# parthjaggi/flow

Measured on AMD Instinct MI355X. Metric: env-steps/sec, higher is better.
Workload: dtype mixed

## Files before the change

flow_amd/csrc/flowsim.hip:

```cpp
#include "flowsim_sim.h"

namespace fsim {

int validate(const fs_config* c) {
  if (!c) return fail(FS_ERR_INVALID, "fs_create: cfg is NULL");
  if (c->struct_size != sizeof(fs_config))
    return fail(FS_ERR_INVALID, "fs_create: struct_size mismatch (header/library out of sync)");
  if (c->abi_version != FS_ABI_VERSION) return fail(FS_ERR_INVALID, "fs_create: abi_version mismatch");
  if (c->precision != FS_F32 && c->precision != FS_F64 && c->precision != FS_MIXED && c->precision != FS_F16S)
    return fail(FS_ERR_INVALID, "fs_create: bad precision");
  if (c->precision == FS_F16S && (c->network != FS_NET_MERGE || c->num_vehicles > 64))
    return fail(FS_ERR_UNSUPPORTED, "fs_create: FS_F16S (half state, float32 integrator) is built for FS_NET_MERGE "
                                    "(k_steps_open, <= 64 vehicle slots)");
  if (c->precision == FS_MIXED && (c->network == FS_NET_MERGE || c->network == FS_NET_BOTTLENECK)) {
  } else if (c->precision == FS_MIXED) {
    const bool fig8 = c->network == FS_NET_FIGURE_EIGHT;
    const char* why = nullptr;
    if ((c->network != FS_NET_RING && !fig8) || c->num_lanes > 1) why = "network (single-lane ring or figure eight)";
    else if (c->env != FS_ENV_ACCEL && c->env != FS_ENV_WAVE_ATTENUATION_PO) why = "env (AccelEnv or WaveAttenuationPOEnv)";
    else if (c->evaluate) why = "evaluate";
    else if (c->sims_per_step != 1) why = "sims_per_step (1)";
    else if (c->integrator != FS_EULER) why = "integrator (Euler)";
    else if (c->junction_mode && !fig8) why = "junction_mode";
    else if (c->track_aux && !fig8) why = "track_aux (the scalar Env's previous-speed / acceleration fields: VecFlowEnv(track_aux=False))";
// ... 334 lines not shown
  return FS_OK;
}

int fs_use_own_stream(fs_handle h) {
  if (!h) return fail(FS_ERR_INVALID, "fs_use_own_stream: NULL handle");
  SimBase* s = S(h);
  DeviceGuard guard(s->cfg.device);
  HIP_TRY(hipStreamSynchronize(s->stream));
  s->stream = s->own_stream;
  return FS_OK;
}

int fs_sync(fs_handle h) {
  if (!h) return fail(FS_ERR_INVALID, "fs_sync: NULL handle");
  DeviceGuard guard(S(h)->cfg.device);
  HIP_TRY(hipStreamSynchronize(S(h)->stream));
  return S(h)->check_qflag();
}

int fs_reset_dev(fs_handle h, const uint8_t* mask_dev, float* obs_dev) {
  if (!h) return fail(FS_ERR_INVALID, "fs_reset_dev: NULL handle");
  SimBase* s = S(h);
  DeviceGuard guard(s->cfg.device);
  int rc = s->launch_reset(mask_dev);
  if (rc) return rc;
  float* obs = obs_dev ? obs_dev : s->d_obs;
  if (s->cfg.network == FS_NET_MERGE || s->cfg.network == FS_NET_BOTTLENECK) {
    s->after_reset = 1;
    rc = s->launch_steps(0, mask_dev, nullptr, 0, obs, s->d_rew, s->d_done, 0);
    s->after_reset = 0;
    if (rc) return rc;
    if (s->cfg.warmup_steps > 0)
      return s->launch_steps(s->cfg.warmup_steps, mask_dev, nullptr, 0, obs, s->d_rew, s->d_done, 0);
    return FS_OK;
  }
  if (s->cfg.warmup_steps > 0)
    return s->launch_steps(s->cfg.warmup_steps, mask_dev, nullptr, 0, obs, s->d_rew, s->d_done, 0);
  return s->launch_steps(0, mask_dev, nullptr, 0, obs, s->d_rew, s->d_done, 0);
}

int fs_reset(fs_handle h, const uint8_t* mask, float* obs_out) {
  if (!h) return fail(FS_ERR_INVALID, "fs_reset: NULL handle");
  SimBase* s = S(h);
  DeviceGuard guard(s->cfg.device);
  const size_t R = size_t(s->cfg.num_replicas);
  const uint8_t* dmask = nullptr;
  if (mask) {
    HIP_TRY(hipMemcpyAsync(s->d_mask, mask, R, hipMemcpyHostToDevice, s->stream));
    dmask = s->d_mask;
// ... 118 lines not shown
```

flow_amd/csrc/flowsim_kernels.h:

```cpp
#pragma once
#include <hip/hip_runtime.h>
#include <stdint.h>

#include "flowsim.h"

namespace fs {

enum : int {
  FLAG_NEED_FOLLOWER = 1,
  FLAG_NEED_MEAN = 2,
  FLAG_HAS_NOISE = 4,
  FLAG_HAS_LAC = 8,
  FLAG_NEED_SUMO = 16,
  FLAG_HAS_FAILSAFE = 32,
  FLAG_ALL_IDM = 64,
  FLAG_IDM_SET = 128,
  FLAG_NO_FLOW_CTRL = 256,
  FLAG_DELTA4 = 512,
};

template <typename T>
struct DevView {
  T* pos;
  T* vel;
// ... 1675 lines not shown
  }

  if (num_steps == 0) {
    write_obs();
    return;
  }

  if (valid && live_replica) {
    s.pos[idx] = x;
    s.vel[idx] = v;
    s.lane[idx] = ln;
    s.last_lc[idx] = last_lc;
    if (sorted) s.sort_key[idx] = xs;
    if (flags & FLAG_HAS_LAC) s.ctrl_state[idx] = cst;
    if (s.track_aux) { s.prev_vel[idx] = prev_v; s.accel[idx] = last_acc; }
    if (ii == 0) {
      s.time[rr] = tcount;
      if (flags & FLAG_HAS_NOISE) s.noise_ctr[rr] = nctr;
    }
  }
}

template <typename T>
__global__ void k_reset(DevView<T> s, const uint8_t* __restrict__ mask) {
  const size_t n = size_t(s.R) * s.N;
  for (size_t e = size_t(blockIdx.x) * blockDim.x + threadIdx.x; e < n; e += size_t(gridDim.x) * blockDim.x) {
    const int r = int(e / s.N);
    if (mask != nullptr && mask[r] == 0) continue;
    s.pos[e] = s.init_pos[e];
    s.vel[e] = s.init_vel[e];
    s.prev_vel[e] = s.init_vel[e];
    s.accel[e] = T(0);
    s.ctrl_state[e] = T(0);
    if (e % s.N == 0 && s.init_ring_len != nullptr) const_cast<T*>(s.ring_len)[r] = s.init_ring_len[r];
    if (s.sort_vehicles) {
      T xa = s.init_pos[e];
      if (s.nseg > 0) {
        bool internal;
        segment_lookup_args(s, s.init_pos[e], internal, xa);
      }
      s.sort_key[e] = xa;
    }
    if (s.num_lanes > 1 || s.env == FS_ENV_LANE_CHANGE_ACCEL || s.env == FS_ENV_LANE_CHANGE_ACCEL_PO) {
      s.lane[e] = s.init_lane[e];
      s.last_lc[e] = -(1 << 30);
    }
    if (s.n_pis > 0 && s.pis_index[e % s.N] >= 0) s.pis_n[size_t(r) * s.n_pis + s.pis_index[e % s.N]] = 0;
    if (e % s.N == 0) s.time[r] = 0;
  }
}

}
```

flow_amd/csrc/flowsim_pair.h:

```cpp
#pragma once
#include "flowsim_kernels.h"

namespace fs {

typedef float f2 __attribute__((ext_vector_type(2)));
typedef unsigned u2v __attribute__((__vector_size__(8)));

enum : int { DPP_ROW_NEWBCAST0 = 0x150, DPP_ROW_NEWBCAST8 = 0x158 };

__device__ __forceinline__ f2 fma2(f2 a, f2 b, f2 c) { return __builtin_elementwise_fma(a, b, c); }
__device__ __forceinline__ f2 splat(float a) { return f2{a, a}; }

__device__ __forceinline__ f2 pk_mul(f2 a, f2 b) { return a * b; }
__device__ __forceinline__ f2 pk_add(f2 a, f2 b) { return a + b; }
__device__ __forceinline__ f2 pk_sub(f2 a, f2 b) { return a - b; }
__device__ __forceinline__ f2 pk_fma(f2 a, f2 b, f2 c) { return fma2(a, b, c); }
__device__ __forceinline__ f2 pk_fnma(f2 a, f2 b, f2 c) { return fma2(-a, b, c); }
__device__ __forceinline__ float nonneg_else(float x, float y) {
  const unsigned a = __builtin_bit_cast(unsigned, x), b = __builtin_bit_cast(unsigned, y);
  return __builtin_bit_cast(float, min(a, b));
}

template <int ROW>
__device__ __forceinline__ float next_a(float v, bool last, int lane) {
// ... 142 lines not shown
      "v_pk_fma_f32 v[124:125], v[112:113], %[vmask], %[tvm]\n"
      "v_pk_mul_f32 v[124:125], v[124:125], v[124:125]\n"
      "v_add_f32_e32 %[sq], v124, v125\n"
      "v_cvt_f64_f32_e32 v[130:131], v112\n"
      "v_cvt_f64_f32_e32 v[132:133], v113\n"
      "v_mul_f64 v[134:135], v[130:131], %[rcms]\n"
      "v_mul_f64 v[136:137], v[132:133], %[rcms]\n"
      "v_fma_f64 v[130:131], -v[134:135], %[ms], v[130:131]\n"
      "v_fma_f64 v[132:133], -v[136:137], %[ms], v[132:133]\n"
      "v_fma_f64 v[134:135], v[130:131], %[rcms], v[134:135]\n"
      "v_fma_f64 v[136:137], v[132:133], %[rcms], v[136:137]\n"
      "v_cvt_f32_f64_e32 v128, v[134:135]\n"
      "v_cvt_f32_f64_e32 v129, v[136:137]\n"
      : "+{v[112:113]}"(V), "+{v[114:115]}"(X), "+{v[116:117]}"(H), "+{v[118:119]}"(DVL), "={v[128:129]}"(OV),
        [cb] "+v"(crash_bits), [sq] "=&v"(sq)
      : [L2] "v"(c.L2), [lenlead] "v"(c.len_lead), [gap2] "v"(c.gap2), [vmask] "v"(c.vmask), [tvm] "v"(c.tvm),
        [ms] "v"(c.ms64), [rcms] "v"(c.rc_ms64), [last] "s"(c.last_mask)
      : "v124", "v125", "v126", "v127", "v130", "v131", "v132", "v133", "v134", "v135", "v136", "v137");
}

struct MixedConsts {
  f2 p0, p1, p2, p5, rc_v0, tsab, rc_ab, one, gap2, vmask, tvm;
  float c1e3;
  double dt, ramp, L, rc_L, rc_ms, len_b, len_next, zero;
  unsigned long long last_mask;
};
__device__ __forceinline__ void mixed_step_asm_a(f2& V32, double& XA, double& XB, double& VA, double& VB, f2& H, f2& DVL,
                                                 f2& OV, const MixedConsts& c) {
  unsigned long long sa, sb;
  asm volatile(
      "v_cmp_nlt_f32_e64 %[sa], |v140|, %[c1e3]\n"
      "v_cmp_nlt_f32_e64 %[sb], |v141|, %[c1e3]\n"
      "v_pk_mul_f32 v[124:125], v[112:113], v[142:143]\n"
      "v_pk_mul_f32 v[126:127], v[124:125], %[rcab]\n"
      "v_pk_fma_f32 v[130:131], v[126:127], %[tsab], v[124:125] neg_lo:[1,0,0] neg_hi:[1,0,0]\n"
      "v_pk_fma_f32 v[126:127], v[130:131], %[rcab], v[126:127]\n"
      "v_cndmask_b32_e64 v120, %[c1e3], v140, %[sa]\n"
      "v_cndmask_b32_e64 v121, %[c1e3], v141, %[sb]\n"
      "v_pk_mul_f32 v[124:125], v[112:113], %[rcv0]\n"
      "v_rcp_f32_e32 v122, v120\n"
      "v_rcp_f32_e32 v123, v121\n"
      "v_pk_fma_f32 v[130:131], v[124:125], %[p0], v[112:113] neg_lo:[1,0,0] neg_hi:[1,0,0]\n"
      "v_pk_fma_f32 v[124:125], v[130:131], %[rcv0], v[124:125]\n"
      "v_pk_mul_f32 v[130:131], v[112:113], %[p1]\n"
      "v_pk_add_f32 v[130:131], v[130:131], v[126:127]\n"
      "v_pk_fma_f32 v[126:127], v[120:121], v[122:123], %[one] neg_lo:[1,0,0] neg_hi:[1,0,0]\n"
      "v_max_f32_e32 v130, 0, v130\n"
      "v_max_f32_e32 v131, 0, v131\n"
      "v_pk_fma_f32 v[122:123], v[126:127], v[122:123], v[122:123]\n"
      "v_pk_add_f32 v[130:131], %[p5], v[130:131]\n"
      "v_pk_mul_f32 v[124:125], v[124:125], v[124:125]\n"
// ... 3 lines not shown
      "v_pk_add_f32 v[124:125], %[one], v[124:125] neg_lo:[0,1] neg_hi:[0,1]\n"
      "v_pk_fma_f32 v[126:127], v[132:133], v[122:123], v[126:127]\n"
      "v_pk_fma_f32 v[132:133], v[120:121], v[126:127], v[130:131] neg_lo:[1,0,0] neg_hi:[1,0,0]\n"
      "v_pk_fma_f32 v[126:127], v[132:133], v[122:123], v[126:127]\n"
      "v_pk_mul_f32 v[126:127], v[126:127], v[126:127]\n"
      "v_pk_add_f32 v[124:125], v[124:125], v[126:127] neg_lo:[0,1] neg_hi:[0,1]\n"
      "v_pk_mul_f32 v[124:125], %[p2], v[124:125]\n"
      "v_cvt_f64_f32_e32 v[130:131], v124\n"
      "v_cvt_f64_f32_e32 v[132:133], v125\n"
      "v_mul_f64 v[130:131], v[130:131], %[dt]\n"
      "v_mul_f64 v[132:133], v[132:133], %[dt]\n"
      "v_add_f64 v[130:131], v[118:119], v[130:131]\n"
      "v_add_f64 v[132:133], v[138:139], v[132:133]\n"
      "v_max_f64 v[130:131], v[130:131], %[zero]\n"
      "v_max_f64 v[132:133], v[132:133], %[zero]\n"
      "v_add_f64 v[130:131], v[130:131], -v[118:119]\n"
      "v_add_f64 v[132:133], v[132:133], -v[138:139]\n"
      "v_mul_f64 v[130:131], v[130:131], %[ramp]\n"
      "v_mul_f64 v[132:133], v[132:133], %[ramp]\n"
      "v_add_f64 v[118:119], v[118:119], v[130:131]\n"
      "v_add_f64 v[138:139], v[138:139], v[132:133]\n"
      "v_mul_f64 v[130:131], v[118:119], %[dt]\n"
      "v_mul_f64 v[132:133], v[138:139], %[dt]\n"
      "v_add_f64 v[130:131], v[114:115], v[130:131]\n"
      "v_add_f64 v[132:133], v[116:117], v[132:133]\n"
      "v_add_f64 v[134:135], v[130:131], -%[L]\n"
      "v_add_f64 v[136:137], v[132:133], -%[L]\n"
      "v_cvt_f32_f64_e32 v112, v[118:119]\n"
      "v_cvt_f32_f64_e32 v113, v[138:139]\n"
      "v_cmp_gt_i32_e64 %[sa], 0, v135\n"
      "v_cmp_gt_i32_e64 %[sb], 0, v137\n"
      "v_mul_f64 v[120:121], v[118:119], %[rcms]\n"
      "v_mul_f64 v[122:123], v[138:139], %[rcms]\n"
      "v_cndmask_b32_e64 v114, v134, v130, %[sa]\n"
      "v_cndmask_b32_e64 v115, v135, v131, %[sa]\n"
      "v_cndmask_b32_e64 v116, v136, v132, %[sb]\n"
      "v_cndmask_b32_e64 v117, v137, v133, %[sb]\n"
      "v_cvt_f32_f64_e32 v128, v[120:121]\n"
      "v_cvt_f32_f64_e32 v129, v[122:123]\n"
      : "+{v[112:113]}"(V32), "+{v[114:115]}"(XA), "+{v[116:117]}"(XB), "+{v[118:119]}"(VA), "+{v[138:139]}"(VB),
        "+{v[140:141]}"(H), "+{v[142:143]}"(DVL), "={v[128:129]}"(OV), [sa] "=&s"(sa), [sb] "=&s"(sb)
      : [c1e3] "v"(c.c1e3), [rcab] "v"(c.rc_ab), [tsab] "v"(c.tsab), [rcv0] "v"(c.rc_v0), [p0] "v"(c.p0),
        [p1] "v"(c.p1), [p2] "v"(c.p2), [p5] "v"(c.p5), [one] "v"(c.one), [dt] "v"(c.dt), [ramp] "v"(c.ramp),
        [L] "v"(c.L), [rcms] "v"(c.rc_ms), [zero] "v"(c.zero)
      : "v120", "v121", "v122", "v123", "v124", "v125", "v126", "v127", "v130", "v131", "v132", "v133", "v134",
        "v135", "v136", "v137");
}
struct MixedSumoConsts { double fl0a, fl0b, adta, adtb, ddta, ddtb; };
__device__ __forceinline__ void mixed_step_asm_a_sm(f2& V32, double& XA, double& XB, double& VA, double& VB, f2& H,
                                                    f2& DVL, f2& OV, const MixedConsts& c, const SumoPair& m,
                                                    const MixedSumoConsts& d) {
  unsigned long long sa, sb;
  asm volatile(
      "v_cmp_nlt_f32_e64 %[sa], |v140|, %[c1e3]\n"
      "v_cmp_nlt_f32_e64 %[sb], |v141|, %[c1e3]\n"
      "v_pk_mul_f32 v[124:125], v[112:113], v[142:143]\n"
      "v_pk_mul_f32 v[126:127], v[124:125], %[rcab]\n"
      "v_pk_mul_f32 v[150:151], v[124:125], %[rcts]\n"
      "v_pk_fma_f32 v[130:131], v[126:127], %[tsab], v[124:125] neg_lo:[1,0,0] neg_hi:[1,0,0]\n"
      "v_pk_fma_f32 v[152:153], v[150:151], %[ts], v[124:125] neg_lo:[1,0,0] neg_hi:[1,0,0]\n"
      "v_pk_fma_f32 v[126:127], v[130:131], %[rcab], v[126:127]\n"
      "v_pk_fma_f32 v[150:151], v[152:153], %[rcts], v[150:151]\n"
      "v_cndmask_b32_e64 v120, %[c1e3], v140, %[sa]\n"
      "v_cndmask_b32_e64 v121, %[c1e3], v141, %[sb]\n"
      "v_max_f32_e32 v146, v140, %[c1e3]\n"
      "v_max_f32_e32 v147, v141, %[c1e3]\n"
      "v_pk_mul_f32 v[124:125], v[112:113], %[rcv0]\n"
      "v_rcp_f32_e32 v122, v120\n"
      "v_rcp_f32_e32 v123, v121\n"
      "v_rcp_f32_e32 v148, v146\n"
      "v_rcp_f32_e32 v149, v147\n"
      "v_pk_fma_f32 v[130:131], v[124:125], %[p0], v[112:113] neg_lo:[1,0,0] neg_hi:[1,0,0]\n"
      "v_pk_mul_f32 v[154:155], v[112:113], %[rcsm]\n"
      "v_pk_fma_f32 v[124:125], v[130:131], %[rcv0], v[124:125]\n"
// ... 49 lines not shown
      "v_add_f64 v[136:137], v[138:139], v[136:137]\n"
      "v_max_f64 v[130:131], v[130:131], %[zero]\n"
      "v_max_f64 v[132:133], v[132:133], %[zero]\n"
      "v_max_f64 v[134:135], v[134:135], %[fl0a]\n"
      "v_max_f64 v[136:137], v[136:137], %[fl0b]\n"
      "v_add_f64 v[130:131], v[130:131], -v[118:119]\n"
      "v_add_f64 v[132:133], v[132:133], -v[138:139]\n"
      "v_mul_f64 v[130:131], v[130:131], %[ramp]\n"
      "v_mul_f64 v[132:133], v[132:133], %[ramp]\n"
      "v_add_f64 v[130:131], v[118:119], v[130:131]\n"
      "v_add_f64 v[132:133], v[138:139], v[132:133]\n"
      "v_min_f64 v[130:131], v[130:131], v[134:135]\n"
      "v_min_f64 v[132:133], v[132:133], v[136:137]\n"
      "v_add_f64 v[134:135], v[118:119], %[adta]\n"
      "v_add_f64 v[136:137], v[138:139], %[adtb]\n"
      "v_min_f64 v[130:131], v[130:131], v[134:135]\n"
      "v_min_f64 v[132:133], v[132:133], v[136:137]\n"
      "v_add_f64 v[134:135], v[118:119], -%[ddta]\n"
      "v_add_f64 v[136:137], v[138:139], -%[ddtb]\n"
      "v_max_f64 v[118:119], v[130:131], v[134:135]\n"
      "v_max_f64 v[138:139], v[132:133], v[136:137]\n"
      "v_mul_f64 v[130:131], v[118:119], %[dt]\n"
      "v_mul_f64 v[132:133], v[138:139], %[dt]\n"
      "v_add_f64 v[130:131], v[114:115], v[130:131]\n"
      "v_add_f64 v[132:133], v[116:117], v[132:133]\n"
      "v_add_f64 v[134:135], v[130:131], -%[L]\n"
      "v_add_f64 v[136:137], v[132:133], -%[L]\n"
      "v_cvt_f32_f64_e32 v112, v[118:119]\n"
      "v_cvt_f32_f64_e32 v113, v[138:139]\n"
      "v_cmp_gt_i32_e64 %[sa], 0, v135\n"
      "v_cmp_gt_i32_e64 %[sb], 0, v137\n"
      "v_mul_f64 v[120:121], v[118:119], %[rcms]\n"
      "v_mul_f64 v[122:123], v[138:139], %[rcms]\n"
      "v_cndmask_b32_e64 v114, v134, v130, %[sa]\n"
      "v_cndmask_b32_e64 v115, v135, v131, %[sa]\n"
      "v_cndmask_b32_e64 v116, v136, v132, %[sb]\n"
      "v_cndmask_b32_e64 v117, v137, v133, %[sb]\n"
      "v_cvt_f32_f64_e32 v128, v[120:121]\n"
      "v_cvt_f32_f64_e32 v129, v[122:123]\n"
      : "+{v[112:113]}"(V32), "+{v[114:115]}"(XA), "+{v[116:117]}"(XB), "+{v[118:119]}"(VA), "+{v[138:139]}"(VB),
        "+{v[140:141]}"(H), "+{v[142:143]}"(DVL), "={v[128:129]}"(OV), [sa] "=&s"(sa), [sb] "=&s"(sb)
      : [c1e3] "v"(c.c1e3), [rcab] "v"(c.rc_ab), [tsab] "v"(c.tsab), [rcv0] "v"(c.rc_v0), [p0] "v"(c.p0),
        [p1] "v"(c.p1), [p2] "v"(c.p2), [p5] "v"(c.p5), [one] "v"(c.one), [dt] "v"(c.dt), [ramp] "v"(c.ramp),
        [L] "v"(c.L), [rcms] "v"(c.rc_ms), [zero] "v"(c.zero), [rcts] "v"(m.rc_ts), [ts] "v"(m.ts),
        [rcsm] "v"(m.rc_smax), [smax] "v"(m.smax), [tau] "v"(m.tau), [mgap] "v"(m.min_gap), [maxa] "v"(m.maxa),
        [fl0a] "v"(d.fl0a), [fl0b] "v"(d.fl0b), [adta] "v"(d.adta), [adtb] "v"(d.adtb), [ddta] "v"(d.ddta),
        [ddtb] "v"(d.ddtb)
      : "v120", "v121", "v122", "v123", "v124", "v125", "v126", "v127", "v130", "v131", "v132", "v133", "v134",
        "v135", "v136", "v137", "v146", "v147", "v148", "v149", "v150", "v151", "v152", "v153", "v154", "v155");
}
__device__ __forceinline__ void mixed_step_asm_b(f2& V32, double& XA, double& XB, f2& H, f2& DVL, f2& OX,
                                                 unsigned& crash_bits, float& sq, const MixedConsts& c) {
  unsigned long long sa, sb;
  asm volatile(
      "v_sub_f32_e32 v142, v112, v113\n"
      "v_subrev_f32_dpp v143, v112, v113 row_shl:1 row_mask:0xf bank_mask:0xf bound_ctrl:1\n"
      "v_subrev_f32_dpp v124, v112, v113 row_newbcast:0 row_mask:0xf bank_mask:0xf\n"
      "v_mov_b32_dpp v130, v114 row_shl:1 row_mask:0xf bank_mask:0xf bound_ctrl:1\n"
      "v_mov_b32_dpp v131, v115 row_shl:1 row_mask:0xf bank_mask:0xf bound_ctrl:1\n"
      "v_mov_b32_dpp v132, v114 row_newbcast:0 row_mask:0xf bank_mask:0xf\n"
      "v_mov_b32_dpp v133, v115 row_newbcast:0 row_mask:0xf bank_mask:0xf\n"
      "v_cndmask_b32_e64 v143, v143, v124, %[last]\n"
      "v_cndmask_b32_e64 v130, v130, v132, %[last]\n"
      "v_cndmask_b32_e64 v131, v131, v133, %[last]\n"
      "v_mul_f64 v[120:121], v[114:115], %[rcL]\n"
      "v_mul_f64 v[122:123], v[116:117], %[rcL]\n"
      "v_add_f64 v[134:135], v[116:117], -v[114:115]\n"
      "v_add_f64 v[136:137], v[130:131], -v[116:117]\n"
      "v_cvt_f32_f64_e32 v144, v[120:121]\n"
      "v_cvt_f32_f64_e32 v145, v[122:123]\n"
      "v_add_f64 v[130:131], v[134:135], %[L]\n"
      "v_add_f64 v[132:133], v[136:137], %[L]\n"
      "v_cmp_gt_i32_e64 %[sa], 0, v135\n"
      "v_cmp_gt_i32_e64 %[sb], 0, v137\n"
      "v_pk_fma_f32 v[124:125], v[112:113], %[vmask], %[tvm]\n"
      "v_pk_mul_f32 v[124:125], v[124:125], v[124:125]\n"
      "v_cndmask_b32_e64 v134, v134, v130, %[sa]\n"
      "v_cndmask_b32_e64 v135, v135, v131, %[sa]\n"
      "v_cndmask_b32_e64 v136, v136, v132, %[sb]\n"
      "v_cndmask_b32_e64 v137, v137, v133, %[sb]\n"
      "v_add_f32_e32 %[sq], v124, v125\n"
      "v_add_f64 v[134:135], v[134:135], -%[lenb]\n"
      "v_add_f64 v[136:137], v[136:137], -%[lennext]\n"
      "v_cvt_f32_f64_e32 v140, v[134:135]\n"
      "v_cvt_f32_f64_e32 v141, v[136:137]\n"
      "v_pk_add_f32 v[126:127], v[140:141], %[gap2] neg_lo:[0,1] neg_hi:[0,1]\n"
      "v_min_f32_e32 v126, v126, v127\n"
      "v_alignbit_b32 %[cb], %[cb], v126, 31\n"
      : "+{v[112:113]}"(V32), "+{v[114:115]}"(XA), "+{v[116:117]}"(XB), "+{v[140:141]}"(H), "+{v[142:143]}"(DVL),
        "={v[144:145]}"(OX), [cb] "+v"(crash_bits), [sq] "=&v"(sq), [sa] "=&s"(sa), [sb] "=&s"(sb)
      : [L] "v"(c.L), [rcL] "v"(c.rc_L), [gap2] "v"(c.gap2), [vmask] "v"(c.vmask), [tvm] "v"(c.tvm),
        [lenb] "v"(c.len_b), [lennext] "v"(c.len_next), [last] "s"(c.last_mask)
      : "v120", "v121", "v122", "v123", "v124", "v125", "v126", "v127", "v130", "v131", "v132", "v133", "v134",
        "v135", "v136", "v137");
}

template <typename T, int ROW, bool DELTA4, bool FASTDIV, bool BADCHK, bool SM = false, bool NOISE = false>
__global__ __launch_bounds__(256) void k_rollout_pair(DevView<T> s, int num_steps, float* __restrict__ obs,
                                                      float* __restrict__ rew, uint8_t* __restrict__ done) {
  constexpr bool MIXED = sizeof(T) == 8;
  static_assert(!(NOISE && MIXED), "FS_MIXED has no noise form (its C twin cannot reproduce the hardware's log / cos)");
  constexpr bool ASM = ROW == 16 && DELTA4 && FASTDIV && !BADCHK;
  constexpr int RPW = 64 / ROW;
  constexpr int PERIOD = ROW < 16 ? ROW : 16;
  const int lane = threadIdx.x & 63;
  const int wave = (blockIdx.x * blockDim.x + threadIdx.x) >> 6;
  const int row = lane / ROW;
  const int k = lane % ROW;
  const int r = wave * RPW + row;
  const int N = s.N;
  const int LP = N >> 1;
  const bool rvalid = r < s.R;
  const bool valid = rvalid && k < LP;
  const int rr = rvalid ? r : s.R - 1;
// ... 17 lines not shown
  if constexpr (NOISE) {
    if ((nctr & 3u) != 0u) {
      gauss4<float>(s.seed_lo, s.seed_hi, s.rep0 + uint32_t(rr), uint32_t(iA), nctr >> 2, gA, s.noise_exact != 0);
      gauss4<float>(s.seed_lo, s.seed_hi, s.rep0 + uint32_t(rr), uint32_t(iB), nctr >> 2, gB, s.noise_exact != 0);
      for (uint32_t q = 0; q < (nctr & 3u); ++q) {
        gA[0] = gA[1]; gA[1] = gA[2]; gA[2] = gA[3];
        gB[0] = gB[1]; gB[1] = gB[2]; gB[2] = gB[3];
      }
    }
  }

  const float dt = float(s.dt), ramp = float(s.ramp);
  const f2 two_sqrt_ab = {2.0f * tsqrt(p[2].x * p[3].x), 2.0f * tsqrt(p[2].y * p[3].y)};
  const f2 rc_v0 = {1.0f / p[0].x, 1.0f / p[0].y}, rc_ab = {1.0f / two_sqrt_ab.x, 1.0f / two_sqrt_ab.y};
  const float Lf = float(L);
  const f2 L2 = splat(Lf), rc_L2 = splat(1.0f / Lf), one = splat(1.0f), dt2 = splat(dt), ramp2 = splat(ramp);
  const f2 gap2 = splat(float(s.crash_gap)), m100 = splat(-100.0f);
  const f2 vmask = splat(valid ? 1.0f : 0.0f), tvm = splat(valid ? -float(s.target_velocity) : 0.0f);
  const double ms64 = double(s.max_speed), rc_ms64 = 1.0 / ms64;
  const double L64 = double(L), rc_L64 = 1.0 / L64, dt64 = double(s.dt), ramp64 = double(s.ramp);

  f2 x, v;
  double xdA = 0, xdB = 0, vdA = 0, vdB = 0;
  if (MIXED) {
    xdA = double(s.pos[idx]); xdB = double(s.pos[idx + 1]);
    vdA = double(s.vel[idx]); vdB = double(s.vel[idx + 1]);
    v = f2{float(vdA), float(vdB)};
    x = f2{0.0f, 0.0f};
  } else {
    x = f2{float(s.pos[idx]), float(s.pos[idx + 1])};
    v = f2{float(s.vel[idx]), float(s.vel[idx + 1])};
  }
  const f2 len_lead = {float(lenB), float(len_nextA)};

  auto headway = [&]() -> f2 {
    if (MIXED) {
      const double xn = next_a<ROW>(xdA, last, lane);
      double dA = xdB - xdA, dB = xn - xdB;
      dA = dA < 0.0 ? dA + L64 : dA;
      dB = dB < 0.0 ? dB + L64 : dB;
      return f2{float(dA - double(lenB)), float(dB - double(len_nextA))};
    } else {
      const f2 xl = {x.y, next_a<ROW>(x.x, last, lane)};
      f2 d = pk_sub(xl, x);
      const f2 dw = pk_add(d, L2);
      d.x = nonneg_else(d.x, dw.x);
      d.y = nonneg_else(d.y, dw.y);
      return pk_sub(d, len_lead);
    }
  };
  f2 h = headway();
  f2 vl = {v.y, next_a<ROW>(v.x, last, lane)};
  f2 dvl = v - vl;
  PairConsts pc;
  pc.p0 = p[0]; pc.p1 = p[1]; pc.p2 = p[2]; pc.p5 = p[5]; pc.rc_v0 = rc_v0; pc.tsab = two_sqrt_ab; pc.rc_ab = rc_ab;
  pc.one = one; pc.dt2 = dt2; pc.ramp2 = ramp2; pc.L2 = L2; pc.rc_L2 = rc_L2; pc.len_lead = len_lead;
  pc.gap2 = gap2; pc.vmask = vmask; pc.tvm = tvm; pc.c1e3 = 1e-3f; pc.ms64 = ms64; pc.rc_ms64 = rc_ms64;
  pc.last_mask = __ballot(last);
  MixedConsts mc;
  mc.p0 = p[0]; mc.p1 = p[1]; mc.p2 = p[2]; mc.p5 = p[5]; mc.rc_v0 = rc_v0; mc.tsab = two_sqrt_ab; mc.rc_ab = rc_ab;
  mc.one = one; mc.gap2 = gap2; mc.vmask = vmask; mc.tvm = tvm; mc.c1e3 = 1e-3f; mc.dt = dt64; mc.ramp = ramp64;
  mc.L = L64; mc.rc_L = rc_L64; mc.rc_ms = rc_ms64; mc.len_b = double(lenB); mc.len_next = double(len_nextA);
  mc.zero = 0.0; mc.last_mask = pc.last_mask;
  SumoPair sc{};
  double floor0A = 0, floor0B = 0, adtA = 0, adtB = 0, ddtA = 0, ddtB = 0;
  if constexpr (SM) {
    const int mA = s.speed_mode[iA], mB = s.speed_mode[iB];
    const float maA = float(s.max_accel[iA]), maB = float(s.max_accel[iB]);
    const float mdA = float(s.max_decel[iA]), mdB = float(s.max_decel[iB]);
    sc.tau = f2{float(s.sumo_tau[iA]), float(s.sumo_tau[iB])};
    sc.min_gap = f2{float(s.sumo_min_gap[iA]), float(s.sumo_min_gap[iB])};
    sc.maxa = f2{maA, maB};
    sc.smax = f2{float(s.sumo_max_speed[iA]), float(s.sumo_max_speed[iB])};
    sc.rc_smax = f2{1.0f / sc.smax.x, 1.0f / sc.smax.y};
    sc.ts = f2{2.0f * tsqrt(maA * mdA), 2.0f * tsqrt(maB * mdB)};
    sc.rc_ts = f2{1.0f / sc.ts.x, 1.0f / sc.ts.y};
    const float BIG = 3.0e38f;
    sc.floor0 = f2{(mA & 1) ? 0.0f : BIG, (mB & 1) ? 0.0f : BIG};
    sc.adt = f2{(mA & 2) ? maA * dt : BIG, (mB & 2) ? maB * dt : BIG};
    sc.ddt = f2{(mA & 4) ? mdA * dt : BIG, (mB & 4) ? mdB * dt : BIG};
    floor0A = double(sc.floor0.x); floor0B = double(sc.floor0.y);
    adtA = (mA & 2) ? double(s.max_accel[iA]) * dt64 : double(BIG);
    adtB = (mB & 2) ? double(s.max_accel[iB]) * dt64 : double(BIG);
    ddtA = (mA & 4) ? double(s.max_decel[iA]) * dt64 : double(BIG);
    ddtB = (mB & 4) ? double(s.max_decel[iB]) * dt64 : double(BIG);
  }
// ... 27 lines not shown
    if constexpr (NOISE) {
      const bool fresh = (nctr & 3u) == 0u;
      if (__ballot(fresh) != 0ull) {
        if (fresh) {
          gauss4<float>(s.seed_lo, s.seed_hi, s.rep0 + uint32_t(rr), uint32_t(iA), nctr >> 2, gA, s.noise_exact != 0);
          gauss4<float>(s.seed_lo, s.seed_hi, s.rep0 + uint32_t(rr), uint32_t(iB), nctr >> 2, gB, s.noise_exact != 0);
        }
      }
      const float tA = sigma.x * gA[0], tB = sigma.y * gB[0];
      nz.x = noisyA ? tA : -0.0f;
      nz.y = noisyB ? tB : -0.0f;
      gA[0] = gA[1]; gA[1] = gA[2]; gA[2] = gA[3];
      gB[0] = gB[1]; gB[1] = gB[2]; gB[2] = gB[3];
      nctr += 1u;
    }
    return nz;
  };

  auto one_step = [&](int slot, __amdgpu_buffer_rsrc_t rs, float& sq_out) {
    if constexpr (ASM) {
      f2 ov, ox;
      const unsigned so = unsigned(slot) * step_b32;
      if constexpr (MIXED) {
        if constexpr (SM) mixed_step_asm_a_sm(v, xdA, xdB, vdA, vdB, h, dvl, ov, mc, sc, msc);
        else mixed_step_asm_a(v, xdA, xdB, vdA, vdB, h, dvl, ov, mc);
        if (slot > 0) __builtin_amdgcn_raw_buffer_store_b128(piece, rs, off_16, so - step_b32, 0);
        mixed_step_asm_b(v, xdA, xdB, h, dvl, ox, crash_bits, sq_out, mc);
        transpose_in(ov, ox);
      } else {
#if defined(FS_DIAG_NOSTORE)
        pair_step_asm_a(v, x, h, dvl, ox, pc);
        pair_step_asm_b(v, x, h, dvl, ov, crash_bits, sq_out, pc);
        asm volatile("" :: "v"(ov), "v"(ox), "s"(so));
#elif defined(FS_DIAG_NOXPOSE)
        pair_step_asm_a(v, x, h, dvl, ox, pc);
        __builtin_amdgcn_raw_buffer_store_b64(__builtin_bit_cast(u2v, ox), rs, off_x, so, 0);
        pair_step_asm_b(v, x, h, dvl, ov, crash_bits, sq_out, pc);
        __builtin_amdgcn_raw_buffer_store_b64(__builtin_bit_cast(u2v, ov), rs, off_v, so, 0);
#else
        if constexpr (NOISE) {
          const f2 nz = noise_term();
          if constexpr (SM) pair_step_asm_a_sm_nz(v, x, h, dvl, ox, pc, sc, nz);
          else pair_step_asm_a_nz(v, x, h, dvl, ox, pc, nz);
        } else {
          if constexpr (SM) pair_step_asm_a_sm(v, x, h, dvl, ox, pc, sc);
          else pair_step_asm_a(v, x, h, dvl, ox, pc);
        }
        if (slot > 0) __builtin_amdgcn_raw_buffer_store_b128(piece, rs, off_16, so - step_b32, 0);
        pair_step_asm_b(v, x, h, dvl, ov, crash_bits, sq_out, pc);
        transpose_in(ov, ox);
// ... 149 lines not shown
```

flow_amd/csrc/flowsim_sim.h:

```cpp
#pragma once
#include <hip/hip_runtime.h>

#include <algorithm>
#include <climits>
#include <cmath>
#include <cstdio>
#include <cstdlib>
#include <cstring>
#include <map>
#include <mutex>
#include <new>
#include <string>
#include <type_traits>
#include <vector>

#include "flowsim.h"
#include "flowsim_kernels.h"
#include "flowsim_open.h"
#include "flowsim_pair.h"
#include "flowsim_fig8.h"
#include "flowsim_ringrl.h"
#include "flowsim_policy.h"
#include "flowsim_wide.h"
#include "flowsim_queue_consts.h"
// ... 68 lines not shown
  int* d_qflag = nullptr;
  bool qflag_armed = false;
  int check_qflag() {
    if (!qflag_armed || !d_qflag) return FS_OK;
    int f = 0;
    HIP_TRY(hipMemcpy(&f, d_qflag, sizeof(int), hipMemcpyDeviceToHost));
    if (f != 0)
      return fail(FS_ERR_UNSUPPORTED, "k_drop_queue: a path of the lane-drop network held more than 64 vehicles (or more than 8 "
                                      "arrived in one sub-step): the results of this handle are invalid -- create it "
                                      "with FLOWSIM_NO_QUEUE=1 (slot-order kernels)");
    qflag_armed = false;
    return FS_OK;
  }
  bool has_user_ctrl = false;
  const char* last_kernel = "";
  int launched() {
    HIP_TRY(hipGetLastError());
    return FS_OK;
  }

  virtual int launch_steps(int num_steps, const uint8_t* mask, const float* actions, size_t act_stride,
                           float* obs, float* rew, uint8_t* done, int obs_every_step) = 0;
  virtual int launch_reset(const uint8_t* mask) = 0;
  virtual int launch_policy(const fs_policy* pol, int num_steps, int reset_done, const float* obs_in, float* obs,
                            float* act, float* logp, float* rew, uint8_t* done) = 0;
  uint32_t* d_pol_ctr = nullptr;
  virtual int get_state(int field, void* dst, size_t bytes) = 0;
  virtual int set_state(int field, const void* src, size_t bytes) = 0;
  virtual int add_vehicle(int replica, int slot, int route, double x, double speed) = 0;
};

template <typename T>
struct Sim : SimBase {
  fs::DevView<T> dv{};
  fs::OpenView<T> ov{};
  fs::QueueConsts qc{};
  bool open_net = false;
  std::vector<T> h_len;
  std::vector<T> h_ring_len;

  template <typename U>
  int dev_alloc(U** out, size_t count) {
    void* p = nullptr;
    HIP_TRY(hipMalloc(&p, (count ? count : 1) * sizeof(U)));
    allocs.push_back(p);
    *out = static_cast<U*>(p);
// ... 758 lines not shown
    if (loop) return launch_policy_loop16(pv, num_steps, reset_done, obs, act, logp, rew, done);
    return launch_policy_row16(pv, num_steps, reset_done, obs, act, logp, rew, done);
  }

  int launch_reset(const uint8_t* mask) override {
    if (mask == nullptr) neg_speed_possible = init_vel_negative;
    if (open_net) {
      const size_t n_open = size_t(dv.R) * dv.N;
      int blocks_open = int((n_open + 255) / 256);
      if (blocks_open > 2048) blocks_open = 2048;
      hipLaunchKernelGGL((fs::k_reset_open<T>), dim3(blocks_open), dim3(256), 0, stream, dv, ov, mask);
      if (dv.st16) hipLaunchKernelGGL((fs::k_state16_pack<T>), dim3(blocks_open), dim3(256), 0, stream, dv, mask);
      HIP_TRY(hipGetLastError());
      return FS_OK;
    }
    const size_t n = size_t(dv.R) * dv.N;
    int blocks = int((n + 255) / 256);
    if (blocks > 2048) blocks = 2048;
    hipLaunchKernelGGL((fs::k_reset<T>), dim3(blocks), dim3(256), 0, stream, dv, mask);
    HIP_TRY(hipGetLastError());
    return FS_OK;
  }

  T* field_ptr(int field, size_t* count, bool* writable) {
    const size_t RN = size_t(dv.R) * dv.N;
    *writable = true;
    switch (field) {
      case FS_FIELD_POS: *count = RN; return dv.pos;
      case FS_FIELD_VEL: *count = RN; return dv.vel;
      case FS_FIELD_PREV_VEL: *count = RN; return dv.prev_vel;
      case FS_FIELD_ACCEL: *count = RN; return dv.accel;
      case FS_FIELD_CTRL_STATE: *count = RN; return dv.ctrl_state;
      case FS_FIELD_MAX_SPEED: *count = open_net ? RN : 0; return open_net ? ov.vmax : nullptr;
      case FS_FIELD_RING_LENGTH: *count = size_t(dv.R); return const_cast<T*>(dv.ring_len);
      case FS_FIELD_INIT_RING_LENGTH: *count = size_t(dv.R); return const_cast<T*>(dv.init_ring_len);
      case FS_FIELD_SORT_KEY: *count = RN; return dv.sort_key;
      case FS_FIELD_INIT_POS: *count = RN; return const_cast<T*>(dv.init_pos);
      case FS_FIELD_INIT_VEL: *count = RN; return const_cast<T*>(dv.init_vel);
      default: *count = 0; return nullptr;
    }
  }

  int get_state(int field, void* dst, size_t bytes) override {
    if (dv.st16 && (field == FS_FIELD_POS || field == FS_FIELD_VEL)) {
      hipLaunchKernelGGL((fs::k_state16_unpack<T>), dim3(256), dim3(256), 0, stream, dv);
      HIP_TRY(hipGetLastError());
// ... 182 lines not shown
```

Before: 13.18 billion.

## Fuse reset with observation write and replace wrap cndmasks with fmac

```diff
diff --git a/flow_amd/csrc/flowsim.hip b/flow_amd/csrc/flowsim.hip
--- a/flow_amd/csrc/flowsim.hip
+++ b/flow_amd/csrc/flowsim.hip
@@ -380,9 +380,10 @@
   if (!h) return fail(FS_ERR_INVALID, "fs_reset_dev: NULL handle");
   SimBase* s = S(h);
   DeviceGuard guard(s->cfg.device);
+  float* obs = obs_dev ? obs_dev : s->d_obs;
+  if (s->reset_obs_ok()) return s->launch_reset_obs(mask_dev, obs);
   int rc = s->launch_reset(mask_dev);
   if (rc) return rc;
-  float* obs = obs_dev ? obs_dev : s->d_obs;
   if (s->cfg.network == FS_NET_MERGE || s->cfg.network == FS_NET_BOTTLENECK) {
     s->after_reset = 1;
     rc = s->launch_steps(0, mask_dev, nullptr, 0, obs, s->d_rew, s->d_done, 0);
diff --git a/flow_amd/csrc/flowsim_kernels.h b/flow_amd/csrc/flowsim_kernels.h
--- a/flow_amd/csrc/flowsim_kernels.h
+++ b/flow_amd/csrc/flowsim_kernels.h
@@ -1721,32 +1721,59 @@
 }
 
 template <typename T>
+__device__ __forceinline__ void reset_element(const DevView<T>& s, size_t e, int r) {
+  s.pos[e] = s.init_pos[e];
+  s.vel[e] = s.init_vel[e];
+  s.prev_vel[e] = s.init_vel[e];
+  s.accel[e] = T(0);
+  s.ctrl_state[e] = T(0);
+  if (e % s.N == 0 && s.init_ring_len != nullptr) const_cast<T*>(s.ring_len)[r] = s.init_ring_len[r];
+  if (s.sort_vehicles) {
+    T xa = s.init_pos[e];
+    if (s.nseg > 0) {
+      bool internal;
+      segment_lookup_args(s, s.init_pos[e], internal, xa);
+    }
+    s.sort_key[e] = xa;
+  }
+  if (s.num_lanes > 1 || s.env == FS_ENV_LANE_CHANGE_ACCEL || s.env == FS_ENV_LANE_CHANGE_ACCEL_PO) {
+    s.lane[e] = s.init_lane[e];
+    s.last_lc[e] = -(1 << 30);
+  }
+  if (s.n_pis > 0 && s.pis_index[e % s.N] >= 0) s.pis_n[size_t(r) * s.n_pis + s.pis_index[e % s.N]] = 0;
+  if (e % s.N == 0) s.time[r] = 0;
+}
+template <typename T>
 __global__ void k_reset(DevView<T> s, const uint8_t* __restrict__ mask) {
   const size_t n = size_t(s.R) * s.N;
   for (size_t e = size_t(blockIdx.x) * blockDim.x + threadIdx.x; e < n; e += size_t(gridDim.x) * blockDim.x) {
     const int r = int(e / s.N);
     if (mask != nullptr && mask[r] == 0) continue;
-    s.pos[e] = s.init_pos[e];
-    s.vel[e] = s.init_vel[e];
-    s.prev_vel[e] = s.init_vel[e];
-    s.accel[e] = T(0);
-    s.ctrl_state[e] = T(0);
-    if (e % s.N == 0 && s.init_ring_len != nullptr) const_cast<T*>(s.ring_len)[r] = s.init_ring_len[r];
-    if (s.sort_vehicles) {
-      T xa = s.init_pos[e];
-      if (s.nseg > 0) {
-        bool internal;
-        segment_lookup_args(s, s.init_pos[e], internal, xa);
-      }
-      s.sort_key[e] = xa;
-    }
-    if (s.num_lanes > 1 || s.env == FS_ENV_LANE_CHANGE_ACCEL || s.env == FS_ENV_LANE_CHANGE_ACCEL_PO) {
-      s.lane[e] = s.init_lane[e];
-      s.last_lc[e] = -(1 << 30);
-    }
-    if (s.n_pis > 0 && s.pis_index[e % s.N] >= 0) s.pis_n[size_t(r) * s.n_pis + s.pis_index[e % s.N]] = 0;
-    if (e % s.N == 0) s.time[r] = 0;
-  }
-}
-
-}
+    reset_element(s, e, r);
+  }
+}
+
+template <typename T>
+__global__ void k_reset_obs(DevView<T> s, const uint8_t* __restrict__ mask, float* __restrict__ obs) {
+  constexpr bool MIXED = sizeof(T) == 8;
+  const size_t n = size_t(s.R) * s.N;
+  const double ms64 = double(s.max_speed), rc_ms64 = 1.0 / ms64;
+  for (size_t e = size_t(blockIdx.x) * blockDim.x + threadIdx.x; e < n; e += size_t(gridDim.x) * blockDim.x) {
+    const int r = int(e / s.N), i = int(e % s.N);
+    const bool selected = mask == nullptr || mask[r] != 0;
+    const T base_len = selected && s.init_ring_len != nullptr ? s.init_ring_len[r] : s.ring_len[r];
+    const T x = selected ? s.init_pos[e] : s.pos[e], v = selected ? s.init_vel[e] : s.vel[e];
+    if (selected) reset_element(s, e, r);
+    const T L = base_len + T(4) * s.jlen;
+    float* o = obs + size_t(r) * 2 * s.N;
+    if (MIXED) {
+      o[i] = float(double(v) * rc_ms64);
+      o[s.N + i] = float(double(x) * (1.0 / double(L)));
+    } else {
+      o[i] = div_via_f64(float(v), ms64, rc_ms64);
+      o[s.N + i] = float(x) / float(L);
+    }
+  }
+}
+
+}
diff --git a/flow_amd/csrc/flowsim_pair.h b/flow_amd/csrc/flowsim_pair.h
--- a/flow_amd/csrc/flowsim_pair.h
+++ b/flow_amd/csrc/flowsim_pair.h
@@ -188,11 +188,12 @@
 struct MixedConsts {
   f2 p0, p1, p2, p5, rc_v0, tsab, rc_ab, one, gap2, vmask, tvm;
   float c1e3;
-  double dt, ramp, L, rc_L, rc_ms, len_b, len_next, zero;
+  double dt, ramp, L, negL, rc_L, rc_ms, len_b, len_next, zero;
+  unsigned onehi;
   unsigned long long last_mask;
 };
 __device__ __forceinline__ void mixed_step_asm_a(f2& V32, double& XA, double& XB, double& VA, double& VB, f2& H, f2& DVL,
-                                                 f2& OV, const MixedConsts& c) {
+                                                 double& WA, double& WB, f2& OV, const MixedConsts& c) {
   unsigned long long sa, sb;
   asm volatile(
       "v_cmp_nlt_f32_e64 %[sa], |v140|, %[c1e3]\n"
@@ -242,34 +243,33 @@
       "v_add_f64 v[138:139], v[138:139], v[132:133]\n"
       "v_mul_f64 v[130:131], v[118:119], %[dt]\n"
       "v_mul_f64 v[132:133], v[138:139], %[dt]\n"
-      "v_add_f64 v[130:131], v[114:115], v[130:131]\n"
-      "v_add_f64 v[132:133], v[116:117], v[132:133]\n"
-      "v_add_f64 v[134:135], v[130:131], -%[L]\n"
-      "v_add_f64 v[136:137], v[132:133], -%[L]\n"
+      "v_add_f64 v[114:115], v[114:115], v[130:131]\n"
+      "v_add_f64 v[116:117], v[116:117], v[132:133]\n"
+      "v_cmp_ge_f64_e64 %[sa], v[114:115], %[L]\n"
+      "v_cmp_ge_f64_e64 %[sb], v[116:117], %[L]\n"
       "v_cvt_f32_f64_e32 v112, v[118:119]\n"
       "v_cvt_f32_f64_e32 v113, v[138:139]\n"
-      "v_cmp_gt_i32_e64 %[sa], 0, v135\n"
-      "v_cmp_gt_i32_e64 %[sb], 0, v137\n"
+      "v_cndmask_b32_e64 v157, 0, %[onehi], %[sa]\n"
+      "v_cndmask_b32_e64 v159, 0, %[onehi], %[sb]\n"
       "v_mul_f64 v[120:121], v[118:119], %[rcms]\n"
+      "v_fmac_f64_e32 v[114:115], %[negL], v[156:157]\n"
+      "v_fmac_f64_e32 v[116:117], %[negL], v[158:159]\n"
       "v_mul_f64 v[122:123], v[138:139], %[rcms]\n"
-      "v_cndmask_b32_e64 v114, v134, v130, %[sa]\n"
-      "v_cndmask_b32_e64 v115, v135, v131, %[sa]\n"
-      "v_cndmask_b32_e64 v116, v136, v132, %[sb]\n"
-      "v_cndmask_b32_e64 v117, v137, v133, %[sb]\n"
       "v_cvt_f32_f64_e32 v128, v[120:121]\n"
       "v_cvt_f32_f64_e32 v129, v[122:123]\n"
       : "+{v[112:113]}"(V32), "+{v[114:115]}"(XA), "+{v[116:117]}"(XB), "+{v[118:119]}"(VA), "+{v[138:139]}"(VB),
-        "+{v[140:141]}"(H), "+{v[142:143]}"(DVL), "={v[128:129]}"(OV), [sa] "=&s"(sa), [sb] "=&s"(sb)
+        "+{v[140:141]}"(H), "+{v[142:143]}"(DVL), "+{v[156:157]}"(WA), "+{v[158:159]}"(WB), "={v[128:129]}"(OV),
+        [sa] "=&s"(sa), [sb] "=&s"(sb)
       : [c1e3] "v"(c.c1e3), [rcab] "v"(c.rc_ab), [tsab] "v"(c.tsab), [rcv0] "v"(c.rc_v0), [p0] "v"(c.p0),
         [p1] "v"(c.p1), [p2] "v"(c.p2), [p5] "v"(c.p5), [one] "v"(c.one), [dt] "v"(c.dt), [ramp] "v"(c.ramp),
-        [L] "v"(c.L), [rcms] "v"(c.rc_ms), [zero] "v"(c.zero)
+        [L] "v"(c.L), [negL] "v"(c.negL), [onehi] "v"(c.onehi), [rcms] "v"(c.rc_ms), [zero] "v"(c.zero)
       : "v120", "v121", "v122", "v123", "v124", "v125", "v126", "v127", "v130", "v131", "v132", "v133", "v134",
         "v135", "v136", "v137");
 }
 struct MixedSumoConsts { double fl0a, fl0b, adta, adtb, ddta, ddtb; };
 __device__ __forceinline__ void mixed_step_asm_a_sm(f2& V32, double& XA, double& XB, double& VA, double& VB, f2& H,
-                                                    f2& DVL, f2& OV, const MixedConsts& c, const SumoPair& m,
-                                                    const MixedSumoConsts& d) {
+                                                    f2& DVL, double& WA, double& WB, f2& OV, const MixedConsts& c,
+                                                    const SumoPair& m, const MixedSumoConsts& d) {
   unsigned long long sa, sb;
   asm volatile(
       "v_cmp_nlt_f32_e64 %[sa], |v140|, %[c1e3]\n"
@@ -365,65 +365,60 @@
       "v_max_f64 v[138:139], v[132:133], v[136:137]\n"
       "v_mul_f64 v[130:131], v[118:119], %[dt]\n"
       "v_mul_f64 v[132:133], v[138:139], %[dt]\n"
-      "v_add_f64 v[130:131], v[114:115], v[130:131]\n"
-      "v_add_f64 v[132:133], v[116:117], v[132:133]\n"
-      "v_add_f64 v[134:135], v[130:131], -%[L]\n"
-      "v_add_f64 v[136:137], v[132:133], -%[L]\n"
+      "v_add_f64 v[114:115], v[114:115], v[130:131]\n"
+      "v_add_f64 v[116:117], v[116:117], v[132:133]\n"
+      "v_cmp_ge_f64_e64 %[sa], v[114:115], %[L]\n"
+      "v_cmp_ge_f64_e64 %[sb], v[116:117], %[L]\n"
       "v_cvt_f32_f64_e32 v112, v[118:119]\n"
       "v_cvt_f32_f64_e32 v113, v[138:139]\n"
-      "v_cmp_gt_i32_e64 %[sa], 0, v135\n"
-      "v_cmp_gt_i32_e64 %[sb], 0, v137\n"
+      "v_cndmask_b32_e64 v157, 0, %[onehi], %[sa]\n"
+      "v_cndmask_b32_e64 v159, 0, %[onehi], %[sb]\n"
       "v_mul_f64 v[120:121], v[118:119], %[rcms]\n"
+      "v_fmac_f64_e32 v[114:115], %[negL], v[156:157]\n"
+      "v_fmac_f64_e32 v[116:117], %[negL], v[158:159]\n"
       "v_mul_f64 v[122:123], v[138:139], %[rcms]\n"
-      "v_cndmask_b32_e64 v114, v134, v130, %[sa]\n"
-      "v_cndmask_b32_e64 v115, v135, v131, %[sa]\n"
-      "v_cndmask_b32_e64 v116, v136, v132, %[sb]\n"
-      "v_cndmask_b32_e64 v117, v137, v133, %[sb]\n"
       "v_cvt_f32_f64_e32 v128, v[120:121]\n"
       "v_cvt_f32_f64_e32 v129, v[122:123]\n"
       : "+{v[112:113]}"(V32), "+{v[114:115]}"(XA), "+{v[116:117]}"(XB), "+{v[118:119]}"(VA), "+{v[138:139]}"(VB),
-        "+{v[140:141]}"(H), "+{v[142:143]}"(DVL), "={v[128:129]}"(OV), [sa] "=&s"(sa), [sb] "=&s"(sb)
+        "+{v[140:141]}"(H), "+{v[142:143]}"(DVL), "+{v[156:157]}"(WA), "+{v[158:159]}"(WB), "={v[128:129]}"(OV),
+        [sa] "=&s"(sa), [sb] "=&s"(sb)
       : [c1e3] "v"(c.c1e3), [rcab] "v"(c.rc_ab), [tsab] "v"(c.tsab), [rcv0] "v"(c.rc_v0), [p0] "v"(c.p0),
         [p1] "v"(c.p1), [p2] "v"(c.p2), [p5] "v"(c.p5), [one] "v"(c.one), [dt] "v"(c.dt), [ramp] "v"(c.ramp),
-        [L] "v"(c.L), [rcms] "v"(c.rc_ms), [zero] "v"(c.zero), [rcts] "v"(m.rc_ts), [ts] "v"(m.ts),
+        [L] "v"(c.L), [negL] "v"(c.negL), [onehi] "v"(c.onehi), [rcms] "v"(c.rc_ms), [zero] "v"(c.zero), [rcts] "v"(m.rc_ts), [ts] "v"(m.ts),
         [rcsm] "v"(m.rc_smax), [smax] "v"(m.smax), [tau] "v"(m.tau), [mgap] "v"(m.min_gap), [maxa] "v"(m.maxa),
         [fl0a] "v"(d.fl0a), [fl0b] "v"(d.fl0b), [adta] "v"(d.adta), [adtb] "v"(d.adtb), [ddta] "v"(d.ddta),
         [ddtb] "v"(d.ddtb)
       : "v120", "v121", "v122", "v123", "v124", "v125", "v126", "v127", "v130", "v131", "v132", "v133", "v134",
         "v135", "v136", "v137", "v146", "v147", "v148", "v149", "v150", "v151", "v152", "v153", "v154", "v155");
 }
-__device__ __forceinline__ void mixed_step_asm_b(f2& V32, double& XA, double& XB, f2& H, f2& DVL, f2& OX,
-                                                 unsigned& crash_bits, float& sq, const MixedConsts& c) {
-  unsigned long long sa, sb;
+__device__ __forceinline__ void mixed_step_asm_b(f2& V32, double& XA, double& XB, f2& H, f2& DVL, double& WA, double& WB,
+                                                 f2& OX, unsigned& crash_bits, float& sq, const MixedConsts& c) {
   asm volatile(
       "v_sub_f32_e32 v142, v112, v113\n"
       "v_subrev_f32_dpp v143, v112, v113 row_shl:1 row_mask:0xf bank_mask:0xf bound_ctrl:1\n"
       "v_subrev_f32_dpp v124, v112, v113 row_newbcast:0 row_mask:0xf bank_mask:0xf\n"
+      "v_mul_f64 v[120:121], v[114:115], %[rcL]\n"
+      "v_mul_f64 v[122:123], v[116:117], %[rcL]\n"
+      "v_add_f64 v[134:135], v[116:117], -v[114:115]\n"
       "v_mov_b32_dpp v130, v114 row_shl:1 row_mask:0xf bank_mask:0xf bound_ctrl:1\n"
       "v_mov_b32_dpp v131, v115 row_shl:1 row_mask:0xf bank_mask:0xf bound_ctrl:1\n"
-      "v_mov_b32_dpp v132, v114 row_newbcast:0 row_mask:0xf bank_mask:0xf\n"
-      "v_mov_b32_dpp v133, v115 row_newbcast:0 row_mask:0xf bank_mask:0xf\n"
+      "v_mov_b64_dpp v[132:133], v[114:115] row_newbcast:0 row_mask:0xf bank_mask:0xf\n"
       "v_cndmask_b32_e64 v143, v143, v124, %[last]\n"
       "v_cndmask_b32_e64 v130, v130, v132, %[last]\n"
       "v_cndmask_b32_e64 v131, v131, v133, %[last]\n"
-      "v_mul_f64 v[120:121], v[114:115], %[rcL]\n"
-      "v_mul_f64 v[122:123], v[116:117], %[rcL]\n"
-      "v_add_f64 v[134:135], v[116:117], -v[114:115]\n"
-      "v_add_f64 v[136:137], v[130:131], -v[116:117]\n"
+      "v_ashrrev_i32_e32 v157, 31, v135\n"
       "v_cvt_f32_f64_e32 v144, v[120:121]\n"
       "v_cvt_f32_f64_e32 v145, v[122:123]\n"
-      "v_add_f64 v[130:131], v[134:135], %[L]\n"
-      "v_add_f64 v[132:133], v[136:137], %[L]\n"
-      "v_cmp_gt_i32_e64 %[sa], 0, v135\n"
-      "v_cmp_gt_i32_e64 %[sb], 0, v137\n"
+      "v_add_f64 v[136:137], v[130:131], -v[116:117]\n"
+      "v_and_b32_e32 v157, %[onehi], v157\n"
       "v_pk_fma_f32 v[124:125], v[112:113], %[vmask], %[tvm]\n"
+      "v_ashrrev_i32_e32 v159, 31, v137\n"
+      "v_fmac_f64_e32 v[134:135], %[L], v[156:157]\n"
+      "v_and_b32_e32 v159, %[onehi], v159\n"
       "v_pk_mul_f32 v[124:125], v[124:125], v[124:125]\n"
-      "v_cndmask_b32_e64 v134, v134, v130, %[sa]\n"
-      "v_cndmask_b32_e64 v135, v135, v131, %[sa]\n"
-      "v_cndmask_b32_e64 v136, v136, v132, %[sb]\n"
-      "v_cndmask_b32_e64 v137, v137, v133, %[sb]\n"
+      "v_fmac_f64_e32 v[136:137], %[L], v[158:159]\n"
+      "v_add_f64 v[134:135], v[134:135], -%[lenb]\n"
       "v_add_f32_e32 %[sq], v124, v125\n"
-      "v_add_f64 v[134:135], v[134:135], -%[lenb]\n"
       "v_add_f64 v[136:137], v[136:137], -%[lennext]\n"
       "v_cvt_f32_f64_e32 v140, v[134:135]\n"
       "v_cvt_f32_f64_e32 v141, v[136:137]\n"
@@ -431,8 +426,8 @@
       "v_min_f32_e32 v126, v126, v127\n"
       "v_alignbit_b32 %[cb], %[cb], v126, 31\n"
       : "+{v[112:113]}"(V32), "+{v[114:115]}"(XA), "+{v[116:117]}"(XB), "+{v[140:141]}"(H), "+{v[142:143]}"(DVL),
-        "={v[144:145]}"(OX), [cb] "+v"(crash_bits), [sq] "=&v"(sq), [sa] "=&s"(sa), [sb] "=&s"(sb)
-      : [L] "v"(c.L), [rcL] "v"(c.rc_L), [gap2] "v"(c.gap2), [vmask] "v"(c.vmask), [tvm] "v"(c.tvm),
+        "+{v[156:157]}"(WA), "+{v[158:159]}"(WB), "={v[144:145]}"(OX), [cb] "+v"(crash_bits), [sq] "=&v"(sq)
+      : [L] "v"(c.L), [rcL] "v"(c.rc_L), [onehi] "v"(c.onehi), [gap2] "v"(c.gap2), [vmask] "v"(c.vmask), [tvm] "v"(c.tvm),
         [lenb] "v"(c.len_b), [lennext] "v"(c.len_next), [last] "s"(c.last_mask)
       : "v120", "v121", "v122", "v123", "v124", "v125", "v126", "v127", "v130", "v131", "v132", "v133", "v134",
         "v135", "v136", "v137");
@@ -496,6 +491,7 @@
 
   f2 x, v;
   double xdA = 0, xdB = 0, vdA = 0, vdB = 0;
+  double wmA = 0.0, wmB = 0.0;
   if (MIXED) {
     xdA = double(s.pos[idx]); xdB = double(s.pos[idx + 1]);
     vdA = double(s.vel[idx]); vdB = double(s.vel[idx + 1]);
@@ -535,7 +531,7 @@
   mc.p0 = p[0]; mc.p1 = p[1]; mc.p2 = p[2]; mc.p5 = p[5]; mc.rc_v0 = rc_v0; mc.tsab = two_sqrt_ab; mc.rc_ab = rc_ab;
   mc.one = one; mc.gap2 = gap2; mc.vmask = vmask; mc.tvm = tvm; mc.c1e3 = 1e-3f; mc.dt = dt64; mc.ramp = ramp64;
   mc.L = L64; mc.rc_L = rc_L64; mc.rc_ms = rc_ms64; mc.len_b = double(lenB); mc.len_next = double(len_nextA);
-  mc.zero = 0.0; mc.last_mask = pc.last_mask;
+  mc.zero = 0.0; mc.last_mask = pc.last_mask; mc.negL = -L64; mc.onehi = 0x3FF00000u;
   SumoPair sc{};
   double floor0A = 0, floor0B = 0, adtA = 0, adtB = 0, ddtA = 0, ddtB = 0;
   if constexpr (SM) {
@@ -609,10 +605,10 @@
       f2 ov, ox;
       const unsigned so = unsigned(slot) * step_b32;
       if constexpr (MIXED) {
-        if constexpr (SM) mixed_step_asm_a_sm(v, xdA, xdB, vdA, vdB, h, dvl, ov, mc, sc, msc);
-        else mixed_step_asm_a(v, xdA, xdB, vdA, vdB, h, dvl, ov, mc);
+        if constexpr (SM) mixed_step_asm_a_sm(v, xdA, xdB, vdA, vdB, h, dvl, wmA, wmB, ov, mc, sc, msc);
+        else mixed_step_asm_a(v, xdA, xdB, vdA, vdB, h, dvl, wmA, wmB, ov, mc);
         if (slot > 0) __builtin_amdgcn_raw_buffer_store_b128(piece, rs, off_16, so - step_b32, 0);
-        mixed_step_asm_b(v, xdA, xdB, h, dvl, ox, crash_bits, sq_out, mc);
+        mixed_step_asm_b(v, xdA, xdB, h, dvl, wmA, wmB, ox, crash_bits, sq_out, mc);
         transpose_in(ov, ox);
       } else {
 #if defined(FS_DIAG_NOSTORE)
diff --git a/flow_amd/csrc/flowsim_sim.h b/flow_amd/csrc/flowsim_sim.h
--- a/flow_amd/csrc/flowsim_sim.h
+++ b/flow_amd/csrc/flowsim_sim.h
@@ -114,6 +114,8 @@
   virtual int launch_steps(int num_steps, const uint8_t* mask, const float* actions, size_t act_stride,
                            float* obs, float* rew, uint8_t* done, int obs_every_step) = 0;
   virtual int launch_reset(const uint8_t* mask) = 0;
+  virtual bool reset_obs_ok() const = 0;
+  virtual int launch_reset_obs(const uint8_t* mask, float* obs) = 0;
   virtual int launch_policy(const fs_policy* pol, int num_steps, int reset_done, const float* obs_in, float* obs,
                             float* act, float* logp, float* rew, uint8_t* done) = 0;
   uint32_t* d_pol_ctr = nullptr;
@@ -918,6 +920,21 @@
     return FS_OK;
   }
 
+  bool reset_obs_ok() const override {
+    const StepArgs a{0, nullptr, nullptr, 0, nullptr, nullptr, nullptr, 0};
+    return cfg.warmup_steps == 0 && !open_net && seg <= 64 && !ml_ok() && !f16s && !has_user_ctrl &&
+           dv.env == FS_ENV_ACCEL && ring_rl_ok(a);
+  }
+  int launch_reset_obs(const uint8_t* mask, float* obs) override {
+    if (mask == nullptr) neg_speed_possible = init_vel_negative;
+    const size_t n = size_t(dv.R) * dv.N;
+    int blocks = int((n + 255) / 256);
+    if (blocks > 2048) blocks = 2048;
+    last_kernel = "k_reset_obs";
+    hipLaunchKernelGGL((fs::k_reset_obs<T>), dim3(blocks), dim3(256), 0, stream, dv, mask, obs);
+    return launched();
+  }
+
   T* field_ptr(int field, size_t* count, bool* writable) {
     const size_t RN = size_t(dv.R) * dv.N;
     *writable = true;
```

Result: slower. 12.83 billion (-2.6%).
